# SelennLamson/AntsRL

Hardware: AMD Instinct MI355X
Metric: ant-steps/sec (ants x envs x steps/s), 256^2 grid (higher is better)
Workload: dtype f64 ant kinematics / f32 grids

## Files before the change

### antsrl_amd/_lib.py

```python
from __future__ import annotations

import ctypes as C
import os

from .config import AntsCfg, AntsGen, AntsInit

LIB_PATH = os.environ.get("ANTSRL_LIB") or os.path.join(os.path.dirname(os.path.abspath(__file__)), "lib",
                                                        "libantsrl_hip.so")

EXPORTS = ("antsrl_abi_version", "antsrl_cfg_size", "antsrl_last_error", "antsrl_workspace_bytes", "antsrl_create",
           "antsrl_destroy", "antsrl_reset", "antsrl_generate", "antsrl_step", "antsrl_observe", "antsrl_update", "antsrl_flush",
           "antsrl_step_update", "antsrl_set_timing_events", "antsrl_set_activation", "antsrl_policy_mlp", "antsrl_read_state", "antsrl_state_bytes",
           "antsrl_set_obs_format", "antsrl_query", "antsrl_bench_copy", "antsrl_set_inloop_policy", "antsrl_set_obs_row_stride", "antsrl_mem_alloc", "antsrl_mem_free",
           "antsrl_mem_trim", "antsrl_mem_stats", "antsrl_update_phase",
           "antsrl_perceptive_field", "antsrl_memnet_packed_bytes", "antsrl_memnet_pack", "antsrl_policy_memory",
           "antsrl_memtrain_sizes", "antsrl_memtrain_init", "antsrl_memtrain_unpack", "antsrl_memtrain_copy",
           "antsrl_memtrain_grad", "antsrl_memtrain_apply", "antsrl_memnet_packed_bytes_ex", "antsrl_memnet_pack_ex",
           "antsrl_policy_memory_ex", "antsrl_agent_select", "antsrl_replay_record_pre", "antsrl_replay_record_post",
           "antsrl_policy_memory_tiles", "antsrl_agent_plan", "antsrl_agent_select_actions",
           "antsrl_replay_record_pre_plain", "antsrl_replay_record_post_plain", "antsrl_lintrain_sizes",
           "antsrl_lintrain_grad", "antsrl_lintrain_apply", "antsrl_lintrain_step", "antsrl_exptrain_sizes",
           "antsrl_exptrain_grad", "antsrl_exptrain_apply", "antsrl_exptrain_step", "antsrl_rework_collapsed_bytes",
           "antsrl_rework_collapse", "antsrl_policy_rework", "antsrl_reworktrain_sizes", "antsrl_reworktrain_grad",
           "antsrl_reworktrain_apply", "antsrl_reworktrain_step", "antsrl_policy_rework_select", "antsrl_monitor_sizes",
           "antsrl_monitor_init", "antsrl_monitor_step", "antsrl_monitor_end_episode")

_lib = None


class AntsMemNetShape(C.Structure):
    _fields_ = [(n, C.c_int32) for n in ("n_features", "agent_dim", "mem_size", "h1", "h2", "h3", "n_rot", "n_ph")]


class AntsReworkShape(C.Structure):
    _fields_ = [(n, C.c_int32) for n in ("n_features", "agent_dim", "g1", "g2", "g3", "r1", "r2", "r3", "p1", "n_rot", "n_ph")]


class AntsRecordSpec(C.Structure):
    _fields_ = [(n, C.c_int32) for n in ("n_envs", "n_ants", "env_id_base", "n_features", "agent_dim", "mem_size", "n_rot",
                                         "obs_format", "obs_pitch", "reserved")] + [
        (n, C.c_int64) for n in ("K", "head", "max_len")] + [(n, C.c_uint64) for n in ("seed", "step")]


class AntsrlError(RuntimeError):
    pass


def load() -> C.CDLL:
    global _lib
    if _lib is not None:
        return _lib
    if not os.path.exists(LIB_PATH):
        raise AntsrlError(
            "libantsrl_hip.so is missing (%s): build it with `python -m antsrl_amd.build` "
            "(hipcc, gfx950).  There is no CPU fallback." % LIB_PATH)
    import torch
    lib = C.CDLL(LIB_PATH)
    vp, i32 = C.c_void_p, C.c_int
    lib.antsrl_abi_version.restype = i32
    lib.antsrl_last_error.restype = C.c_char_p
    lib.antsrl_workspace_bytes.argtypes = [C.POINTER(AntsCfg), C.POINTER(C.c_size_t)]
    lib.antsrl_create.argtypes = [C.POINTER(AntsCfg), vp, C.c_size_t, C.POINTER(vp)]
    lib.antsrl_destroy.argtypes = [vp]
    lib.antsrl_destroy.restype = None
    lib.antsrl_reset.argtypes = [vp, C.POINTER(AntsInit), vp]
    lib.antsrl_generate.argtypes = [vp, C.POINTER(AntsGen), C.c_uint64, vp]
    lib.antsrl_step.argtypes = [vp, vp, vp, vp, vp, vp, vp, vp]
    lib.antsrl_observe.argtypes = [vp, vp, vp, vp, vp]
    lib.antsrl_update.argtypes = [vp, vp, vp]
    lib.antsrl_flush.argtypes = [vp, vp]
    lib.antsrl_update_phase.argtypes = [vp, i32, vp, vp]
    lib.antsrl_perceptive_field.argtypes = [vp, vp, vp]
    lib.antsrl_step_update.argtypes = [vp, vp, vp, vp, vp, vp, vp, vp, vp]
    lib.antsrl_set_timing_events.argtypes = [vp, C.POINTER(vp)]
    lib.antsrl_set_activation.argtypes = [vp, vp, C.c_double, vp]
    lib.antsrl_policy_mlp.argtypes = [vp, vp, vp, C.c_int64, C.c_int32, vp, vp, vp, vp, vp, vp, vp, vp, vp, vp]
    lib.antsrl_read_state.argtypes = [vp, i32, vp, vp]
    lib.antsrl_state_bytes.argtypes = [vp, i32, C.POINTER(C.c_size_t)]
    lib.antsrl_query.argtypes = [vp, i32, C.POINTER(C.c_longlong)]
    lib.antsrl_set_inloop_policy.argtypes = [vp, i32] + [vp] * 9
    lib.antsrl_bench_copy.argtypes = [vp, vp, C.c_size_t, vp]
    lib.antsrl_set_obs_row_stride.argtypes = [vp, i32]
    lib.antsrl_mem_alloc.argtypes = [C.c_size_t, i32, C.POINTER(vp)]
    lib.antsrl_mem_free.argtypes = [vp]
    lib.antsrl_mem_trim.argtypes = []
    lib.antsrl_mem_stats.argtypes = [C.POINTER(C.c_size_t)] * 4
    lib.antsrl_memnet_packed_bytes.argtypes = [C.POINTER(AntsMemNetShape), C.POINTER(C.c_size_t)]
    lib.antsrl_memnet_pack.argtypes = [C.POINTER(AntsMemNetShape), C.POINTER(vp), vp, vp]
    lib.antsrl_policy_memory.argtypes = [C.POINTER(AntsMemNetShape), vp, vp, i32, vp, vp, C.c_int64, vp, vp, vp, vp, vp]
    lib.antsrl_memnet_packed_bytes_ex.argtypes = [C.POINTER(AntsMemNetShape), i32, C.POINTER(C.c_size_t)]
    lib.antsrl_memnet_pack_ex.argtypes = [C.POINTER(AntsMemNetShape), i32, C.POINTER(vp), vp, vp]
    lib.antsrl_policy_memory_ex.argtypes = [C.POINTER(AntsMemNetShape), i32, vp, vp, i32, vp, vp, C.c_int64, vp, vp, vp,
                                            vp, vp]
    lib.antsrl_policy_memory_tiles.argtypes = [C.POINTER(AntsMemNetShape), i32, vp, vp, i32, vp, vp, C.c_int64, vp, vp, vp,
                                               vp, vp, vp, vp]
# ... 100 lines not shown
```

### antsrl_amd/batched.py

```python
from __future__ import annotations

import ctypes as C
from typing import Dict, Optional

import numpy as np
import torch

from . import _lib
from . import config as cfgmod
from . import vmm
from .config import AntsCfg, AntsInit

_STATE_DTYPES = {
    cfgmod.S_ANTS_XYT: torch.float64, cfgmod.S_PREV_XY: torch.float64, cfgmod.S_HOLDING: torch.float32,
    cfgmod.S_MANDIBLES: torch.uint8, cfgmod.S_ACTIVATION: torch.float32, cfgmod.S_PHERO: torch.float32,
    cfgmod.S_FOOD: torch.float32, cfgmod.S_EXPLORED: torch.uint8, cfgmod.S_ANTHILL_FOOD: torch.float64,
    cfgmod.S_ROCK_CENTERS: torch.float64, cfgmod.S_TIMESTEP: torch.int32, cfgmod.S_REWARD_STATE: torch.uint8,
    cfgmod.S_WALLS: torch.uint8, cfgmod.S_ANTHILL_AREA: torch.uint8, cfgmod.S_SEED: torch.float32,
    cfgmod.S_ANTHILL_XYR: torch.int32, cfgmod.S_ROCK_RW: torch.float64,
    cfgmod.S_PHERO_C0: torch.float32, cfgmod.S_PHERO_C1: torch.float32, cfgmod.S_PHERO_C2: torch.float32,
    cfgmod.S_PHERO_C3: torch.float32,
}


import contextlib

_NULL_CTX = contextlib.nullcontext()
_RAW_STREAM = getattr(torch._C, "_cuda_getCurrentRawStream", None)


def _ptr(t: Optional[torch.Tensor]):
    return None if t is None else C.c_void_p(t.data_ptr())


def placement_levels_seen(times) -> bool:
    ok = [t for t in times if t < 1.25 * min(times)]
    return max(ok) >= 1.06 * min(ok)


class BatchedAntsEnv:
    def __init__(self, cfg: AntsCfg, device: Optional[torch.device] = None, obs_dtype: torch.dtype = torch.float32,
                 obs_row_stride=None, pieced_memory: bool = True):
        if obs_dtype not in (torch.float32, torch.bfloat16):
            raise ValueError("obs_dtype must be torch.float32 or torch.bfloat16")
        if not torch.cuda.is_available():
            raise _lib.AntsrlError("BatchedAntsEnv needs an MI355X (torch.cuda.is_available() is False); "
                                   "there is no CPU fallback")
        self.lib = _lib.load()
        self.cfg = cfg.copy()
        self.device = torch.device(device if device is not None else "cuda:%d" % torch.cuda.current_device())
        self._dev_index = self.device.index if self.device.index is not None else torch.cuda.current_device()
        need = C.c_size_t()
        _lib.check(self.lib.antsrl_workspace_bytes(C.byref(self.cfg), C.byref(need)), "workspace_bytes")
        self.workspace_bytes = need.value
        with torch.cuda.device(self.device):
            big = (lambda n: vmm.empty_u8(n, self.device)) if pieced_memory else (lambda n: torch.empty(n, dtype=torch.uint8, device=self.device))
            self._pieced = bool(pieced_memory)
            self._h = None
            self._make_handle(torch.empty(need.value + 256, dtype=torch.uint8, device=self.device))
            E, N, P, K = cfg.n_envs, cfg.n_ants, cfg.pside, cfg.n_channels
            esz = 4 if obs_dtype == torch.float32 else 2
            row = P * P * K
            if obs_row_stride not in (None, "line"):
                raise ValueError("obs_row_stride must be None or 'line'")
            pitch = row if obs_row_stride is None else (row * esz + 127) // 128 * 128 // esz
            sizes = [("agent_state", E * N * 2 * 4), ("reward", E * N * 4), ("done", E), ("obs", E * N * pitch * esz)]
            offs, total = {}, 0
            for name, nbytes in sizes:
                offs[name] = total
                total += (nbytes + 255) // 256 * 256
            self._out_sizes, self._out_offs, self._out_total, self._small_bytes = sizes, offs, total, offs["obs"]
            self._obs_dtype, self._obs_pitch_row = obs_dtype, (pitch, row)
            if obs_dtype == torch.bfloat16:
                _lib.check(self.lib.antsrl_set_obs_format(self._h, 1), "set_obs_format")
            if pitch != row:
                _lib.check(self.lib.antsrl_set_obs_row_stride(self._h, pitch), "set_obs_row_stride")
            self.obs_row_pitch = pitch
            self._bind_outputs(big(total + 256).zero_())
        self._keep = None
        self._loaded = None
        self._host_out = None
        self._host_act = None
        self._act_event = None

    def __del__(self):
        h = getattr(self, "_h", None)
        if h:
            self.lib.antsrl_destroy(h)
            self._h = None

    def _bind_outputs(self, flat: torch.Tensor) -> None:
        c = self.cfg
        E, N, P, K = c.n_envs, c.n_ants, c.pside, c.n_channels
        sizes, offs, total = self._out_sizes, self._out_offs, self._out_total
        pitch, row = self._obs_pitch_row
        base = (-flat.data_ptr()) % 256
        self._out_flat = flat[base:base + total]

        def piece(name, nbytes, dtype, shape):
            return self._out_flat[offs[name]:offs[name] + nbytes].view(dtype).view(shape)
        if pitch == row:
            self.obs = piece("obs", sizes[3][1], self._obs_dtype, (E, N, P, P, K))
            self.obs_padded = None
        else:
            self.obs_padded = piece("obs", sizes[3][1], self._obs_dtype, (E, N, pitch))
            self.obs = self.obs_padded[..., :row].unflatten(-1, (P, P, K))
        self.agent_state = piece("agent_state", sizes[0][1], torch.float32, (E, N, 2))
        self.reward = piece("reward", sizes[1][1], torch.float32, (E, N))
        self.done = piece("done", sizes[2][1], torch.uint8, (E,))
        self._host_out = None

    def _make_handle(self, ws: torch.Tensor) -> None:
        if getattr(self, "_h", None):
            self.lib.antsrl_destroy(self._h)
        self._ws = ws
        self._ws_ptr = ws.data_ptr() + (-ws.data_ptr()) % 256
        self._h = C.c_void_p()
        _lib.check(self.lib.antsrl_create(C.byref(self.cfg), C.c_void_p(self._ws_ptr), self.workspace_bytes, C.byref(self._h)), "create")
        if getattr(self, "_obs_dtype", torch.float32) == torch.bfloat16:
            _lib.check(self.lib.antsrl_set_obs_format(self._h, 1), "set_obs_format")
        pitch, row = getattr(self, "_obs_pitch_row", (0, 0))
        if pitch != row:
            _lib.check(self.lib.antsrl_set_obs_row_stride(self._h, pitch), "set_obs_row_stride")

    def tune_placement(self, age: int = 150, steps: int = 30, verbose: bool = False, extra_outputs: int = 4,
                       walk_spacers: int = 3, spacer_gib: float = 24.0, force_walk: bool = False):
        if self._out_total < vmm.SMALL_BYTES:
            return None
        if self._loaded:
            raise _lib.AntsrlError("tune_placement() must run right after construction: this handle has already been %s" % self._loaded)
        c = self.cfg
        E, N = c.n_envs, c.n_ants
        dev = self.device

        def torch_u8(n):
            return torch.empty(n, dtype=torch.uint8, device=dev)
        with torch.cuda.device(dev):
            g = torch.Generator(device=dev)
            g.manual_seed(7)
            rot = torch.randint(-1, 2, (4, E, N), generator=g, device=dev, dtype=torch.int8)
            ph = torch.randint(0, 3, (4, E, N), generator=g, device=dev, dtype=torch.int8) if c.n_phero == 2 else [None] * 4
            e0, e1 = torch.cuda.Event(enable_timing=True), torch.cuda.Event(enable_timing=True)

            def scratch_episode():
                self.generate(cfgmod.make_gen(), episode_seed=0x7A11)
                for t in range(age):
                    self.step_update(rot[t % 4], ph[t % 4], None)

            NEV, PSTEPS = cfgmod.TIMING_EVENTS, 8
            evs = _lib.HipEvents(NEV * PSTEPS)
            prc_times = []

            def measure():
                for t in range(4):
                    self.step_update(rot[t % 4], ph[t % 4], None)
                e0.record()
                for t in range(steps):
                    self.step_update(rot[t % 4], ph[t % 4], None)
                e1.record()
                for t in range(PSTEPS):
                    self.set_timing_events([evs.ev[NEV * t + i].value for i in range(NEV)])
                    self.step_update(rot[t % 4], ph[t % 4], None)
                torch.cuda.current_stream(dev).synchronize()
                prc_times.append(float(np.mean([evs.elapsed_ms(NEV * t + 2, NEV * t + 3) for t in range(PSTEPS)])))
                return e0.elapsed_time(e1) / steps
            own_ws, own_out = self._ws, self._out_flat
            n_ws, n_out = self.workspace_bytes + 256, self._out_total + 256
            pairs, times = [], []
            for ws_kind in ("own", "other"):
                if ws_kind == "other":
                    self._make_handle(vmm.empty_u8(n_ws, dev))
                scratch_episode()
                for out_kind in ("own", "other"):
                    if out_kind == "other":
                        self._bind_outputs((torch_u8(n_out) if self._pieced else vmm.empty_u8(n_out, dev)).zero_())
                    elif ws_kind == "other":
                        self._bind_outputs(own_out)
                    pairs.append((self._ws, self._out_flat))
                    times.append(measure())
            labels = ["ws torch / out %s" % ("pieced" if self._pieced else "torch"),
                      "ws torch / out %s" % ("torch" if self._pieced else "pieced"),
                      "ws pieced / out %s" % ("pieced" if self._pieced else "torch"),
                      "ws pieced / out %s" % ("torch" if self._pieced else "pieced")]
            if extra_outputs > 0 and self._pieced:
                self._make_handle(own_ws)
                scratch_episode()
                for k in range(int(extra_outputs)):
                    self._bind_outputs(vmm.empty_u8(n_out, dev).zero_())
                    pairs.append((self._ws, self._out_flat))
                    times.append(measure())
                    labels.append("ws torch / out pieced (draw %d)" % (k + 2))
            spacers = []
            walked = 0
            both_levels = placement_levels_seen
            while self._pieced and walked < int(walk_spacers) and (force_walk or not both_levels(prc_times)):
                free_b = torch.cuda.mem_get_info(dev)[0]
                want = int(min(spacer_gib * 2 ** 30, free_b / 5))
                if want < (4 << 30):
                    break
                try:
                    spacers.append(torch_u8(want))
                    spacers.append(vmm.empty_u8(want, dev))
                except (RuntimeError, _lib.AntsrlError):
                    break
                walked += 1
                depth = sum(x.numel() for x in spacers) / 2 ** 30
                if self._ws.data_ptr() != own_ws.data_ptr():
                    self._make_handle(own_ws)
                scratch_episode()
                for kind, mk in (("pieced", lambda: vmm.empty_u8(n_out, dev)), ("torch", lambda: torch_u8(n_out))):
                    self._bind_outputs(mk().zero_())
                    pairs.append((self._ws, self._out_flat))
                    times.append(measure())
                    labels.append("ws torch / out %s (walk %d: +%.0f GiB)" % (kind, walked, depth))
                self._make_handle(torch_u8(n_ws))
                scratch_episode()
                self._bind_outputs(own_out)
                pairs.append((self._ws, self._out_flat))
                times.append(measure())
                labels.append("ws torch (walk %d: +%.0f GiB) / out %s" % (walked, depth, "pieced" if self._pieced else "torch"))
            best = min(range(len(times)), key=prc_times.__getitem__)
            evs.destroy()
            if verbose:
                print("tune_placement: ms/step per (workspace, outputs) pair %s -> %d" % (["%.4f" % t for t in times], best))
            ws, out = pairs[best]
            del pairs, spacers
            if ws.data_ptr() != self._ws.data_ptr():
                self._make_handle(ws)
            self._bind_outputs(out)
            if walked:
                vmm.trim()
            torch.cuda.empty_cache()
            self._out_flat.zero_()
            del own_ws, own_out, ws, out
        self.placement_trials = dict(ms_per_step=[round(t, 5) for t in times], observation_kernel_ms=[round(t, 5) for t in prc_times],
                                     chosen=best, pairs=labels, both_levels_seen=bool(both_levels(prc_times)), walk_steps=walked)
        self._loaded = None
        return times

    @property
    def _obs_buf(self):
        return self.obs if self.obs_padded is None else self.obs_padded

    def _stream(self):
        if _RAW_STREAM is not None:
            return C.c_void_p(_RAW_STREAM(self._dev_index))
        return C.c_void_p(torch.cuda.current_stream(self.device).cuda_stream)

    def _on_device(self):
        return _NULL_CTX if torch.cuda.current_device() == self._dev_index else torch.cuda.device(self.device)

    def _dev(self, a, dtype, shape=None):
        if a is None:
            return None
        t = torch.as_tensor(np.ascontiguousarray(a) if isinstance(a, np.ndarray) else a)
        t = t.to(device=self.device, dtype=dtype).contiguous()
        if shape is not None:
            assert tuple(t.shape) == tuple(shape), "expected shape %s, got %s" % (shape, tuple(t.shape))
        return t

    def reset(self, init: Dict[str, object]) -> None:
        c = self.cfg
        E, N, W, H, Cn, R = c.n_envs, c.n_ants, c.w, c.h, c.n_phero, c.n_rocks
        t = dict(
            ants_xyt=self._dev(init["ants_xyt"], torch.float64, (E, N, 3)),
            seed=self._dev(init["seed"], torch.float64, (E, N)),
            walls=self._dev(init["walls"], torch.uint8, (E, W, H)),
            food=self._dev(init["food"], torch.float32, (E, W, H)),
            anthill_xyr=self._dev(init["anthill_xyr"], torch.int32, (E, 3)),
# ... 189 lines not shown
```

### antsrl_amd/csrc/antsrl_capi.hip

```cpp
#include <hip/hip_runtime.h>
#include <stdarg.h>
#include <stdio.h>
#include <math.h>
#include <stdlib.h>
#include <string.h>
#include <new>

#include "antsrl_device.h"
#include "antsrl_fail.h"

hipError_t antsrl_launch_act(const KP &p, const int8_t *rot, const int8_t *ph, int cur, float *obs,
                             float *agent_state, float *reward, uint8_t *done, int flags, hipStream_t st);
bool antsrl_act_fits(const KP &p);
bool antsrl_act_needs_hbm_maps(const KP &p);
hipError_t antsrl_launch_sweep(const KP &p, int cur, hipStream_t st);
hipError_t antsrl_launch_update(const KP &p, const double *jitter, int out_buf, hipStream_t st, int phases = 15);
hipError_t antsrl_launch_collect_full(const KP &p, hipStream_t st);
hipError_t antsrl_launch_reset(const KP &p, const AntsInit *in, hipStream_t st);
hipError_t antsrl_launch_set_activation(const KP &p, const float *act, hipStream_t st);
hipError_t antsrl_launch_read_state(const KP &p, int which, int cur, void *dst, hipStream_t st);
hipError_t antsrl_launch_perceptive_field(const KP &p, uint8_t *dst, hipStream_t st);
hipError_t antsrl_launch_generate(const KP &p, const AntsGen &g, uint64_t seed, hipStream_t st);
hipError_t antsrl_launch_phero_wall_clear(const KP &p, hipStream_t st, int buf = 0);
hipError_t antsrl_launch_phero_renorm(const KP &p, hipStream_t st);
bool antsrl_meta_supported(const KP &p);
hipError_t antsrl_launch_move(const KP &p, const int8_t *rot, const int8_t *ph, uint8_t *done, int do_step, uint32_t seq,
                              hipStream_t st);
hipError_t antsrl_launch_perceive(const KP &p, int cur, float *obs, float *agent_state, float *reward, int flags,
                                  uint32_t seq, hipStream_t st, const PolArgs *pol, uint32_t obs_pitch);
bool antsrl_inloop_policy_supported(const KP &p);
hipError_t antsrl_launch_policy_pack(unsigned char *pack, const float *w1, const float *b1, const float *w2, const float *b2,
                                     const float *w3, const float *b3, int F, hipStream_t st);
hipError_t antsrl_launch_meta_rebase(const KP &p, hipStream_t st);
bool antsrl_update_move_supported(const KP &p);
hipError_t antsrl_launch_update_move(const KP &p, int out_buf, double g_dep, double inv_g_dep, const int8_t *rot,
                                     const int8_t *ph, uint8_t *done, uint32_t seq, hipStream_t st, bool with_frames);
int antsrl_perceive_run(const KP &p);
hipError_t antsrl_launch_copy16(void *dst, const void *src, size_t bytes, hipStream_t st);

struct AntsHandle {
    AntsCfg cfg;
    KP p;
    int cur;
    int steps_since_update;
    bool need_full_collect;
    bool is_reset;
    bool episode_over;
    size_t ws_bytes;
    AntsGen gen;
    bool has_gen;
    uint64_t episode_seed;
    int host_timestep;
    long long sweeps;
    bool obs_bf16;
    uint32_t obs_pitch;
    bool need_wall_clear;
    hipEvent_t ev[ANTSRL_TIMING_EVENTS];
    bool ev_armed;
    uint32_t obs_seq;
    PolArgs pol;
    bool pend_update;
    KP pend_p;
    int pend_out_buf;
    int phase_next;
};

static thread_local char g_err[512] = "";

int fail(int code, const char *fmt, ...)
{
    va_list ap;
    va_start(ap, fmt);
    vsnprintf(g_err, sizeof(g_err), fmt, ap);
    va_end(ap);
    return code;
}

int hip_fail(hipError_t e, const char *what)
{
    return fail(ANTSRL_E_DEVICE, "%s: %s", what, hipGetErrorString(e));
}
// ... 34 lines not shown
    if (c->filter_radius < 0 || c->filter_radius > ANTSRL_MAX_FILTER_RADIUS)
        return fail(ANTSRL_E_INVALID, "filter_radius must be in 0..%d", ANTSRL_MAX_FILTER_RADIUS);
    if (c->reward_kind < ANTSRL_REWARD_NONE || c->reward_kind > ANTSRL_REWARD_ALL)
        return fail(ANTSRL_E_INVALID, "bad reward_kind");
    if (c->has_max_val && !(c->phero_max_val > 0)) return fail(ANTSRL_E_INVALID, "phero_max_val must be > 0");
    if (c->act_path < ANTSRL_ACT_AUTO || c->act_path > ANTSRL_ACT_SINGLE_KERNEL) return fail(ANTSRL_E_INVALID, "bad act_path");
    if (c->env_id_base < 0 || (long long)c->env_id_base + c->n_envs > 0x7fffffffll)
        return fail(ANTSRL_E_INVALID, "env_id_base must be >= 0 and env_id_base + n_envs must fit 31 bits");
    if (c->n_envs_total != 0 && (long long)c->n_envs_total < (long long)c->env_id_base + c->n_envs)
        return fail(ANTSRL_E_INVALID, "n_envs_total %d < env_id_base + n_envs = %lld (0 = that sum)", c->n_envs_total,
                    (long long)c->env_id_base + c->n_envs);
    if (c->act_path == ANTSRL_ACT_CELL_META) {
        KP kp;
        fill_kp(c, &kp);
        if (!kp.meta)
            return fail(ANTSRL_E_UNSUPPORTED, "ANTSRL_ACT_CELL_META needs 2 pheromone channels, the generator's channel order "
                                              "([Ants, Phero0, Phero1, Anthill, Walls, Food(, Rocks)]), a perception of 128..368 values "
                                              "per ant over at most 64 cells, and at most 4096 ants per env");
    }
    return ANTSRL_OK;
}

static bool use_scaled(const AntsCfg *c)
{
    return c->phero_mode == ANTSRL_PHERO_AUTO && c->filter_radius == 0 && c->filter[0] > 0.5 &&
           c->filter[0] <= 1.0 && c->phero_threshold >= 0.0;
}

static bool use_interleaved(const AntsCfg *c)
{
    return use_scaled(c) && c->n_phero == 2;
}

static size_t carve(const AntsCfg *c, DState *s, unsigned char *base)
{
    const size_t E = c->n_envs, N = c->n_ants, G = (size_t)c->w * c->h, Cn = c->n_phero, R = c->n_rocks;
    const size_t words = (G + 31) / 32;
    size_t off = 0;
    auto take = [&](size_t bytes) -> unsigned char * {
        unsigned char *ptr = base ? base + off : nullptr;
        off = (off + bytes + 255) / 256 * 256;
        return ptr;
    };
    KP kp;
    fill_kp(c, &kp);
    DState d;
    d.x = (double *)take(8 * E * N); d.y = (double *)take(8 * E * N); d.theta = (double *)take(8 * E * N);
    d.prev_x = (double *)take(8 * E * N); d.prev_y = (double *)take(8 * E * N);
    d.prev_dist = (double *)take(8 * E * N);
    d.holding = (float *)take(4 * E * N); d.seed = (float *)take(4 * E * N);
    d.prev_holding = (float *)take(4 * E * N);
    d.activation = (float *)take(4 * E * N * Cn);
    d.mandibles = (uint8_t *)take(E * N); d.reward_state = (uint8_t *)take(E * N);
    d.dirty_cell = (int32_t *)take(4 * E * N);
    d.walldep_cell = (int32_t *)take(4 * E * N);
    if (use_interleaved(c)) {
        d.phero[0] = d.phero[1] = (float *)take(16 * E * G);
        d.food = d.phero[0] ? d.phero[0] + 2 : nullptr;
    } else {
        d.phero[0] = (float *)take(4 * E * G * Cn);
        d.phero[1] = use_scaled(c) ? d.phero[0] : (float *)take(4 * E * G * Cn);
        d.food = (float *)take(4 * E * G * (size_t)kp.fs);
    }
    d.walls_bits = (uint32_t *)take(4 * E * words); d.area_bits = (uint32_t *)take(4 * E * words);
    d.explored_bits = (uint32_t *)take(4 * E * words);
    d.big_pres = d.big_old = nullptr;
    if (!kp.meta && antsrl_act_needs_hbm_maps(kp)) {
        d.big_pres = (uint32_t *)take(4 * E * words);
        d.big_old = (uint32_t *)take(4 * E * words);
    }
    d.primed_cur = kp.meta ? (uint8_t *)take(E) : nullptr;
    d.frames = kp.meta ? (AntFrame *)take(sizeof(AntFrame) * E * N) : nullptr;
    d.anthill_xyr = (int32_t *)take(4 * E * 3);
    d.anthill_food = (double *)take(8 * E);
    d.rock_cx = (double *)take(8 * E * (R ? R : 1)); d.rock_cy = (double *)take(8 * E * (R ? R : 1));
    d.rock_r = (double *)take(8 * E * (R ? R : 1)); d.rock_w = (double *)take(8 * E * (R ? R : 1));
    d.timestep = (int32_t *)take(4 * E);
    d.reward_primed = (uint8_t *)take(E);
    d.gen_discs = (int32_t *)take(4 * E * ANTSRL_MAX_FOOD_DISCS * 3);
    d.gen_perlin = (int32_t *)take(4 * E * 2);
    d.pol_pack = (unsigned char *)take(ANTSRL_POL_PACK_BYTES);
    if (s) *s = d;
    return off;
}

static void fill_kp(const AntsCfg *c, KP *p)
{
    memset(p, 0, sizeof(*p));
    p->E = c->n_envs; p->N = c->n_ants; p->W = c->w; p->H = c->h; p->C = c->n_phero; p->R = c->n_rocks;
    p->K = c->n_channels; p->r = c->perception_radius; p->P = 2 * p->r + 1; p->PP = p->P * p->P;
    p->words = (int)(((size_t)c->w * c->h + 31) / 32);
    int ht = 64;
    while (ht < 2 * c->n_ants) ht <<= 1;
    p->HT = ht;
    p->has_mask = c->has_mask; p->has_max_val = c->has_max_val; p->reward_kind = c->reward_kind;
    p->max_time = c->max_time; p->filter_radius = c->filter_radius;
    p->explore_on = c->reward_kind == ANTSRL_REWARD_EXPLORATION ||
                    (c->reward_kind == ANTSRL_REWARD_ALL &&
                     (c->fct_explore != 0.0 || c->fct_explore_holding != 0.0));
    for (int k = 0; k < ANTSRL_MAX_CHANNELS; ++k) {
        p->ch_kind[k] = c->channel_kind[k];
        p->ch_arg[k] = c->channel_arg[k];
    }
    p->mand_first = p->mand_last = 0;
    for (int k = 0; k < c->n_channels; ++k) {
        const int op = c->channel_kind[k] == ANTSRL_CH_FOOD ? 1 : c->channel_kind[k] == ANTSRL_CH_ANTHILL ? 2 : 0;
        if (op && op != p->mand_last) {
            p->mand_first = p->mand_last;
            p->mand_last = op;
        }
    }
    memcpy(p->mask, c->mask, ANTSRL_MAX_PCELLS);
    p->delta = c->delta; p->fwd_delta = c->fwd_delta; p->max_speed = c->max_speed;
    p->max_rot_speed = c->max_rot_speed; p->carry = c->carry_speed_reduction;
    p->backward = c->backward_speed_reduction; p->max_hold = c->max_hold;
    p->max_val = c->phero_max_val; p->deposit_strength = c->deposit_strength;
// ... 33 lines not shown
                    const float uh = (float)u[k], vh = (float)v[k];
                    p->fsep_u[2 * k] = uh; p->fsep_u[2 * k + 1] = (float)(u[k] - (double)uh);
                    p->fsep_v[2 * k] = vh; p->fsep_v[2 * k + 1] = (float)(v[k] - (double)vh);
                }
            }
        }
    }
    p->rng_seed = c->rng_seed;
    p->env_id_base = (uint32_t)c->env_id_base;
    p->scaled = use_scaled(c) ? 1 : 0;
    p->ps = use_interleaved(c) ? 4 : c->n_phero;
    p->fs = use_interleaved(c) ? 4 : 1;
    p->g_now = p->g_dep = p->inv_g_dep = 1.0;
    p->meta = antsrl_meta_supported(*p) && c->act_path != ANTSRL_ACT_SINGLE_KERNEL ? 1 : 0;
    if (p->meta && p->fs == 1) p->fs = 2;
    p->tiled = (p->meta && p->ps == 4 && p->fs == 4 && (c->w & 1) == 0 && (c->h & 3) == 0) ? 1 : 0;
    p->ftile = (p->meta && p->fs == 2 && (c->w & 3) == 0 && (c->h & 3) == 0) ? 1 : 0;
}

static void set_decay(AntsHandle *h)
{
    if (!h->p.scaled) return;
    const double f0 = h->cfg.filter[0];
    h->p.g_now = pow(f0, (double)h->sweeps);
    h->p.g_dep = pow(f0, (double)(h->sweeps + 1));
    h->p.inv_g_dep = 1.0 / h->p.g_dep;
}

extern "C" int antsrl_workspace_bytes(const AntsCfg *cfg, size_t *bytes)
{
    int rc = validate(cfg);
    if (rc) return rc;
    if (!bytes) return fail(ANTSRL_E_INVALID, "bytes is NULL");
    *bytes = carve(cfg, nullptr, nullptr);
    return ANTSRL_OK;
}

extern "C" int antsrl_create(const AntsCfg *cfg, void *workspace, size_t workspace_bytes, AntsHandle **out)
{
    int rc = validate(cfg);
    if (rc) return rc;
    if (!out) return fail(ANTSRL_E_INVALID, "out is NULL");
    if (!workspace) return fail(ANTSRL_E_INVALID, "workspace is NULL");
    if (((uintptr_t)workspace & 255) != 0) return fail(ANTSRL_E_INVALID, "workspace must be 256-byte aligned");
    const size_t need = carve(cfg, nullptr, nullptr);
    if (workspace_bytes < need)
        return fail(ANTSRL_E_NOMEM, "workspace too small: %zu < %zu bytes", workspace_bytes, need);
    AntsHandle *h = new (std::nothrow) AntsHandle();
    if (!h) return fail(ANTSRL_E_NOMEM, "out of host memory");
    h->cfg = *cfg;
    fill_kp(cfg, &h->p);
    carve(cfg, &h->p.s, (unsigned char *)workspace);
    h->cur = 0; h->steps_since_update = 0; h->need_full_collect = true; h->is_reset = false; h->episode_over = false; h->pend_update = false;
    h->phase_next = 0;
    h->pol = PolArgs{};
    h->sweeps = 0; h->need_wall_clear = false;
    h->has_gen = false; h->episode_seed = 0; h->host_timestep = 1; h->obs_bf16 = false; h->obs_pitch = 0;
    h->ws_bytes = need;
    h->ev_armed = false;
    h->obs_seq = 0;
    if (!h->p.meta && !antsrl_act_fits(h->p)) {
        delete h;
        return fail(ANTSRL_E_UNSUPPORTED,
                    "%d ants with a %dx%d perception need more than 160 KiB of LDS per workgroup "
                    "(per-ant frames, the collision hash and the row staging are kept in LDS)", cfg->n_ants,
                    2 * cfg->perception_radius + 1, 2 * cfg->perception_radius + 1);
    }
    *out = h;
    return ANTSRL_OK;
}

extern "C" void antsrl_destroy(AntsHandle *h) { delete h; }

extern "C" int antsrl_reset(AntsHandle *h, const AntsInit *init, void *stream)
{
    if (!h || !init) return fail(ANTSRL_E_INVALID, "NULL handle or init");
    if (!init->ants_xyt || !init->seed || !init->walls || !init->food || !init->anthill_xyr)
        return fail(ANTSRL_E_INVALID, "AntsInit: ants_xyt, seed, walls, food, anthill_xyr are required");
    if (h->p.R > 0 && !init->rocks) return fail(ANTSRL_E_INVALID, "AntsInit.rocks is NULL but n_rocks > 0");
    h->pend_update = false;
    h->phase_next = 0;
    hipError_t e = antsrl_launch_reset(h->p, init, (hipStream_t)stream);
    if (e != hipSuccess) return hip_fail(e, "reset");
    h->p.deposit_strength = h->cfg.deposit_strength;
    h->cur = 0; h->steps_since_update = 0; h->need_full_collect = true; h->is_reset = true; h->episode_over = false;
    h->sweeps = 0; h->need_wall_clear = h->p.scaled && init->phero != nullptr;
    h->host_timestep = 1; h->obs_seq = 0;
    set_decay(h);
    return ANTSRL_OK;
}

static int check_gen_seed(const AntsHandle *h, const AntsGen &g, uint64_t seed)
{
    const uint64_t top = (uint64_t)h->p.env_id_base + (uint64_t)h->p.E;
    const uint64_t lim = 0xFFFFFFFFull / 5u;
    if (g.rng_kind == ANTSRL_RNG_REFERENCE && (top > lim || seed > lim - top))
        return fail(ANTSRL_E_INVALID, "ANTSRL_RNG_REFERENCE: (episode_seed + env_id_base + n_envs) * 5 must stay below 2^32 (np.random.seed)");
    return ANTSRL_OK;
}

static int do_generate(AntsHandle *h, uint64_t seed, hipStream_t st)
{
// ... 500 lines not shown
```

### include/antsrl.h

```cpp
#ifndef ANTSRL_H
#define ANTSRL_H

#include <stddef.h>
#include <stdint.h>

#ifdef __cplusplus
extern "C" {
#endif

#define ANTSRL_ABI_VERSION 5

#define ANTSRL_MAX_CHANNELS 16
#define ANTSRL_MAX_PSIDE 15
#define ANTSRL_MAX_PCELLS (ANTSRL_MAX_PSIDE * ANTSRL_MAX_PSIDE)
#define ANTSRL_MAX_FILTER_RADIUS 3
#define ANTSRL_MAX_FILTER_TAPS 49
#define ANTSRL_MAX_PHERO 4

#define ANTSRL_OK 0
#define ANTSRL_E_INVALID (-1)
#define ANTSRL_E_NOMEM (-2)
#define ANTSRL_E_DEVICE (-3)
#define ANTSRL_E_UNSUPPORTED (-4)

// ... 98 lines not shown
    ANTSRL_S_PREV_XY = 1,
    ANTSRL_S_HOLDING = 2,
    ANTSRL_S_MANDIBLES = 3,
    ANTSRL_S_ACTIVATION = 4,
    ANTSRL_S_PHERO = 5,
    ANTSRL_S_FOOD = 6,
    ANTSRL_S_EXPLORED = 7,
    ANTSRL_S_ANTHILL_FOOD = 8,
    ANTSRL_S_ROCK_CENTERS = 9,
    ANTSRL_S_TIMESTEP = 10,
    ANTSRL_S_REWARD_STATE = 11,
    ANTSRL_S_WALLS = 12,
    ANTSRL_S_ANTHILL_AREA = 13,
    ANTSRL_S_SEED = 14,
    ANTSRL_S_ANTHILL_XYR = 15,
    ANTSRL_S_ROCK_RW = 16,
    ANTSRL_S_PHERO_C0 = 17,
    ANTSRL_S_PHERO_C1 = 18,
    ANTSRL_S_PHERO_C2 = 19,
    ANTSRL_S_PHERO_C3 = 20,
    ANTSRL_S_COUNT_
};

int antsrl_abi_version(void);

size_t antsrl_cfg_size(void);

const char *antsrl_last_error(void);

int antsrl_workspace_bytes(const AntsCfg *cfg, size_t *bytes);

int antsrl_create(const AntsCfg *cfg, void *workspace, size_t workspace_bytes, AntsHandle **out);

void antsrl_destroy(AntsHandle *h);

int antsrl_reset(AntsHandle *h, const AntsInit *init, void *stream);

int antsrl_generate(AntsHandle *h, const AntsGen *gen, uint64_t episode_seed, void *stream);

int antsrl_step(AntsHandle *h, const int8_t *rotation, const int8_t *phero, float *obs,
                float *agent_state, float *reward, uint8_t *done, void *stream);

int antsrl_observe(AntsHandle *h, float *obs, float *agent_state, float *reward, void *stream);

int antsrl_update(AntsHandle *h, const double *wall_jitter, void *stream);

enum { ANTSRL_PHASE_WALLS = 0, ANTSRL_PHASE_ROCKS_PHEROMONE = 1, ANTSRL_PHASE_ANTS = 2, ANTSRL_PHASE_ANTHILL = 3 };
int antsrl_update_phase(AntsHandle *h, int phase, const double *wall_jitter, void *stream);

int antsrl_flush(AntsHandle *h, void *stream);

int antsrl_step_update(AntsHandle *h, const int8_t *rotation, const int8_t *phero,
                       const double *wall_jitter, float *obs, float *agent_state, float *reward,
                       uint8_t *done, void *stream);

#define ANTSRL_TIMING_EVENTS 5
int antsrl_set_timing_events(AntsHandle *h, void *const *events);

enum {
    ANTSRL_Q_CELL_META = 0,
    ANTSRL_Q_SCALED_UNITS = 1,
    ANTSRL_Q_INTERLEAVED = 2,
    ANTSRL_Q_FILTER_SEPARABLE = 3,
    ANTSRL_Q_PERCEIVE_RUN = 4,
    ANTSRL_Q_TIMESTEP = 5,
    ANTSRL_Q_DEFERRED_UPDATE = 6,
// ... 197 lines not shown
```

Baseline: 2.678 billion.

## Split workspace into separate state and record blocks with tuned placement

Splits the device workspace into two allocations: a small per-ant and per-env state block, and a large record block holding the pheromone and food grids. tune_placement gains a second stage that times alternative placements of the state block (default torch, pieced VMM, or spare record-block candidates). It keeps one only if the update kernel gets faster by a margin. The aim is to cut memory-placement interference between small state arrays and the large grid arrays. It adds API surface and tuning time, and the choice rests on noisy measurements.

```diff
diff --git a/antsrl_amd/_lib.py b/antsrl_amd/_lib.py
--- a/antsrl_amd/_lib.py
+++ b/antsrl_amd/_lib.py
@@ -9,6 +9,7 @@
                                                         "libantsrl_hip.so")
 
 EXPORTS = ("antsrl_abi_version", "antsrl_cfg_size", "antsrl_last_error", "antsrl_workspace_bytes", "antsrl_create",
+           "antsrl_workspace_map",
            "antsrl_destroy", "antsrl_reset", "antsrl_generate", "antsrl_step", "antsrl_observe", "antsrl_update", "antsrl_flush",
            "antsrl_step_update", "antsrl_set_timing_events", "antsrl_set_activation", "antsrl_policy_mlp", "antsrl_read_state", "antsrl_state_bytes",
            "antsrl_set_obs_format", "antsrl_query", "antsrl_bench_copy", "antsrl_set_inloop_policy", "antsrl_set_obs_row_stride", "antsrl_mem_alloc", "antsrl_mem_free",
@@ -42,6 +43,10 @@
         (n, C.c_int64) for n in ("K", "head", "max_len")] + [(n, C.c_uint64) for n in ("seed", "step")]
 
 
+class AntsWsArray(C.Structure):
+    _fields_ = [("name", C.c_char * 24), ("block", C.c_int32), ("_pad", C.c_int32), ("offset", C.c_uint64), ("bytes", C.c_uint64)]
+
+
 class AntsrlError(RuntimeError):
     pass
 
@@ -61,6 +66,9 @@
     lib.antsrl_last_error.restype = C.c_char_p
     lib.antsrl_workspace_bytes.argtypes = [C.POINTER(AntsCfg), C.POINTER(C.c_size_t)]
     lib.antsrl_create.argtypes = [C.POINTER(AntsCfg), vp, C.c_size_t, C.POINTER(vp)]
+    lib.antsrl_workspace_bytes2.argtypes = [C.POINTER(AntsCfg), C.POINTER(C.c_size_t), C.POINTER(C.c_size_t)]
+    lib.antsrl_create2.argtypes = [C.POINTER(AntsCfg), vp, C.c_size_t, vp, C.c_size_t, C.POINTER(vp)]
+    lib.antsrl_workspace_map.argtypes = [C.POINTER(AntsCfg), i32, C.POINTER(AntsWsArray), C.c_int32, C.POINTER(C.c_int32)]
     lib.antsrl_destroy.argtypes = [vp]
     lib.antsrl_destroy.restype = None
     lib.antsrl_reset.argtypes = [vp, C.POINTER(AntsInit), vp]
diff --git a/antsrl_amd/batched.py b/antsrl_amd/batched.py
--- a/antsrl_amd/batched.py
+++ b/antsrl_amd/batched.py
@@ -40,7 +40,7 @@
 
 class BatchedAntsEnv:
     def __init__(self, cfg: AntsCfg, device: Optional[torch.device] = None, obs_dtype: torch.dtype = torch.float32,
-                 obs_row_stride=None, pieced_memory: bool = True):
+                 obs_row_stride=None, pieced_memory: bool = True, split_workspace: bool = True):
         if obs_dtype not in (torch.float32, torch.bfloat16):
             raise ValueError("obs_dtype must be torch.float32 or torch.bfloat16")
         if not torch.cuda.is_available():
@@ -53,11 +53,18 @@
         need = C.c_size_t()
         _lib.check(self.lib.antsrl_workspace_bytes(C.byref(self.cfg), C.byref(need)), "workspace_bytes")
         self.workspace_bytes = need.value
+        nst, nrec = C.c_size_t(), C.c_size_t()
+        _lib.check(self.lib.antsrl_workspace_bytes2(C.byref(self.cfg), C.byref(nst), C.byref(nrec)), "workspace_bytes2")
+        self.state_bytes, self.record_bytes = nst.value, nrec.value
+        self._split = bool(split_workspace)
+        if not self._split:
+            self.state_bytes, self.record_bytes = 0, self.workspace_bytes
         with torch.cuda.device(self.device):
             big = (lambda n: vmm.empty_u8(n, self.device)) if pieced_memory else (lambda n: torch.empty(n, dtype=torch.uint8, device=self.device))
             self._pieced = bool(pieced_memory)
             self._h = None
-            self._make_handle(torch.empty(need.value + 256, dtype=torch.uint8, device=self.device))
+            self._state = None
+            self._make_handle(torch.empty(self.record_bytes + 256, dtype=torch.uint8, device=self.device))
             E, N, P, K = cfg.n_envs, cfg.n_ants, cfg.pside, cfg.n_channels
             esz = 4 if obs_dtype == torch.float32 else 2
             row = P * P * K
@@ -110,13 +117,26 @@
         self.done = piece("done", sizes[2][1], torch.uint8, (E,))
         self._host_out = None
 
-    def _make_handle(self, ws: torch.Tensor) -> None:
+    def _make_handle(self, ws: torch.Tensor, state: Optional[torch.Tensor] = None) -> None:
         if getattr(self, "_h", None):
             self.lib.antsrl_destroy(self._h)
-        self._ws = ws
+            self._h = None
+        if ws.numel() < self.record_bytes + (-ws.data_ptr()) % 256:
+            raise _lib.AntsrlError("record block too small: %d bytes for %d" % (ws.numel(), self.record_bytes))
         self._ws_ptr = ws.data_ptr() + (-ws.data_ptr()) % 256
         self._h = C.c_void_p()
-        _lib.check(self.lib.antsrl_create(C.byref(self.cfg), C.c_void_p(self._ws_ptr), self.workspace_bytes, C.byref(self._h)), "create")
+        if not self._split:
+            self._ws, self._state = ws, None
+            _lib.check(self.lib.antsrl_create(C.byref(self.cfg), C.c_void_p(self._ws_ptr), self.workspace_bytes, C.byref(self._h)), "create")
+        else:
+            if state is None:
+                state = self._state if self._state is not None else torch.empty(self.state_bytes + 256, dtype=torch.uint8, device=self.device)
+            if state.numel() < self.state_bytes + (-state.data_ptr()) % 256:
+                raise _lib.AntsrlError("state block too small: %d bytes for %d" % (state.numel(), self.state_bytes))
+            self._ws, self._state = ws, state
+            self._state_ptr = state.data_ptr() + (-state.data_ptr()) % 256
+            _lib.check(self.lib.antsrl_create2(C.byref(self.cfg), C.c_void_p(self._state_ptr), self.state_bytes,
+                                               C.c_void_p(self._ws_ptr), self.record_bytes, C.byref(self._h)), "create2")
         if getattr(self, "_obs_dtype", torch.float32) == torch.bfloat16:
             _lib.check(self.lib.antsrl_set_obs_format(self._h, 1), "set_obs_format")
         pitch, row = getattr(self, "_obs_pitch_row", (0, 0))
@@ -124,7 +144,7 @@
             _lib.check(self.lib.antsrl_set_obs_row_stride(self._h, pitch), "set_obs_row_stride")
 
     def tune_placement(self, age: int = 150, steps: int = 30, verbose: bool = False, extra_outputs: int = 4,
-                       walk_spacers: int = 3, spacer_gib: float = 24.0, force_walk: bool = False):
+                       walk_spacers: int = 3, spacer_gib: float = 24.0, force_walk: bool = False, state_stage: bool = True):
         if self._out_total < vmm.SMALL_BYTES:
             return None
         if self._loaded:
@@ -147,25 +167,27 @@
                 for t in range(age):
                     self.step_update(rot[t % 4], ph[t % 4], None)
 
-            NEV, PSTEPS = cfgmod.TIMING_EVENTS, 8
-            evs = _lib.HipEvents(NEV * PSTEPS)
+            NEV, PSTEPS, PSTEPS_STATE = cfgmod.TIMING_EVENTS, 8, 24
+            evs = _lib.HipEvents(NEV * PSTEPS_STATE)
             prc_times = []
-
-            def measure():
+            upd_times = []
+
+            def measure(psteps=PSTEPS):
                 for t in range(4):
                     self.step_update(rot[t % 4], ph[t % 4], None)
                 e0.record()
                 for t in range(steps):
                     self.step_update(rot[t % 4], ph[t % 4], None)
                 e1.record()
-                for t in range(PSTEPS):
+                for t in range(psteps):
                     self.set_timing_events([evs.ev[NEV * t + i].value for i in range(NEV)])
                     self.step_update(rot[t % 4], ph[t % 4], None)
                 torch.cuda.current_stream(dev).synchronize()
-                prc_times.append(float(np.mean([evs.elapsed_ms(NEV * t + 2, NEV * t + 3) for t in range(PSTEPS)])))
+                prc_times.append(float(np.mean([evs.elapsed_ms(NEV * t + 2, NEV * t + 3) for t in range(psteps)])))
+                upd_times.append(float(np.mean([evs.elapsed_ms(NEV * t + 1, NEV * t + 2) for t in range(psteps)])))
                 return e0.elapsed_time(e1) / steps
-            own_ws, own_out = self._ws, self._out_flat
-            n_ws, n_out = self.workspace_bytes + 256, self._out_total + 256
+            own_ws, own_out, own_state = self._ws, self._out_flat, self._state
+            n_ws, n_out, n_state = self.record_bytes + 256, self._out_total + 256, self.state_bytes + 256
             pairs, times = [], []
             for ws_kind in ("own", "other"):
                 if ws_kind == "other":
@@ -220,21 +242,52 @@
                 times.append(measure())
                 labels.append("ws torch (walk %d: +%.0f GiB) / out %s" % (walked, depth, "pieced" if self._pieced else "torch"))
             best = min(range(len(times)), key=prc_times.__getitem__)
-            evs.destroy()
             if verbose:
                 print("tune_placement: ms/step per (workspace, outputs) pair %s -> %d" % (["%.4f" % t for t in times], best))
             ws, out = pairs[best]
-            del pairs, spacers
-            if ws.data_ptr() != self._ws.data_ptr():
-                self._make_handle(ws)
+            n_stage1 = len(times)
+            state_cands = [("state torch (default)", own_state)]
+            if state_stage and self._split:
+                try:
+                    state_cands.append(("state pieced", vmm.pieced_u8(n_state, dev)))
+                except _lib.AntsrlError:
+                    pass
+                seen = {ws.data_ptr()}
+                for (w2, _o), lab in zip(pairs, labels):
+                    if w2.data_ptr() not in seen and w2.numel() >= n_state and len(state_cands) < 4:
+                        seen.add(w2.data_ptr())
+                        state_cands.append(("state in spare record block (%s)" % lab.split(" / ")[0], w2[:n_state]))
+            for lab, st in state_cands if len(state_cands) > 1 else []:
+                self._make_handle(ws, st)
+                self._bind_outputs(out)
+                scratch_episode()
+                times.append(measure(PSTEPS_STATE))
+            evs.destroy()
+            s_upd, s_prc = upd_times[n_stage1:], prc_times[n_stage1:]
+            times, prc_times, upd_times = times[:n_stage1], prc_times[:n_stage1], upd_times[:n_stage1]
+            s_best = 0
+            if s_upd:
+                def fast(k, by):
+                    return s_upd[k] <= (1.0 - by) * s_upd[0] and s_upd[k] + s_prc[k] < s_upd[0] + s_prc[0]
+                own = [k for k in range(1, len(s_upd)) if state_cands[k][0] == "state pieced" and fast(k, 0.03)]
+                corners = [k for k in range(1, len(s_upd)) if state_cands[k][0] != "state pieced" and fast(k, 0.05)]
+                if own or corners:
+                    s_best = min(own or corners, key=s_upd.__getitem__)
+            state = state_cands[s_best][1]
+            state_labels = [lab for lab, _ in state_cands]
+            del pairs, spacers, state_cands
+            if ws.data_ptr() != self._ws.data_ptr() or (state is not None and state.data_ptr() != self._state.data_ptr()):
+                self._make_handle(ws, state)
             self._bind_outputs(out)
             if walked:
                 vmm.trim()
             torch.cuda.empty_cache()
             self._out_flat.zero_()
-            del own_ws, own_out, ws, out
+            del own_ws, own_out, own_state, ws, out, state
         self.placement_trials = dict(ms_per_step=[round(t, 5) for t in times], observation_kernel_ms=[round(t, 5) for t in prc_times],
-                                     chosen=best, pairs=labels, both_levels_seen=bool(both_levels(prc_times)), walk_steps=walked)
+                                     chosen=best, pairs=labels, both_levels_seen=bool(both_levels(prc_times)), walk_steps=walked,
+                                     state_stage=dict(candidates=state_labels, update_move_kernel_ms=[round(t, 5) for t in s_upd],
+                                                      observation_kernel_ms=[round(t, 5) for t in s_prc], chosen=s_best))
         self._loaded = None
         return times
 
diff --git a/antsrl_amd/csrc/antsrl_capi.hip b/antsrl_amd/csrc/antsrl_capi.hip
--- a/antsrl_amd/csrc/antsrl_capi.hip
+++ b/antsrl_amd/csrc/antsrl_capi.hip
@@ -46,7 +46,7 @@
     bool need_full_collect;
     bool is_reset;
     bool episode_over;
-    size_t ws_bytes;
+    size_t ws_bytes[2];
     AntsGen gen;
     bool has_gen;
     uint64_t episode_seed;
@@ -147,56 +147,70 @@
     return use_scaled(c) && c->n_phero == 2;
 }
 
-static size_t carve(const AntsCfg *c, DState *s, unsigned char *base)
+static void carve(const AntsCfg *c, DState *s, unsigned char *base, unsigned char *rec_base, bool split, size_t bytes[2],
+                  AntsWsArray *map = nullptr, int32_t cap = 0, int32_t *count = nullptr)
 {
     const size_t E = c->n_envs, N = c->n_ants, G = (size_t)c->w * c->h, Cn = c->n_phero, R = c->n_rocks;
     const size_t words = (G + 31) / 32;
-    size_t off = 0;
-    auto take = [&](size_t bytes) -> unsigned char * {
-        unsigned char *ptr = base ? base + off : nullptr;
-        off = (off + bytes + 255) / 256 * 256;
+    size_t off[2] = {0, 0};
+    int32_t n_arrays = 0;
+    auto take_from = [&](int block, const char *name, size_t nbytes) -> unsigned char * {
+        unsigned char *b = block ? rec_base : base;
+        size_t &o = off[split ? block : 0];
+        unsigned char *ptr = b ? b + o : nullptr;
+        if (map && n_arrays < cap) {
+            AntsWsArray &a = map[n_arrays];
+            memset(&a, 0, sizeof(a));
+            strncpy(a.name, name, sizeof(a.name) - 1);
+            a.block = split ? block : 0; a.offset = o; a.bytes = nbytes;
+        }
+        ++n_arrays;
+        o = (o + nbytes + 255) / 256 * 256;
         return ptr;
     };
+    auto take = [&](const char *name, size_t nbytes) { return take_from(0, name, nbytes); };
+    auto take_rec = [&](const char *name, size_t nbytes) { return take_from(1, name, nbytes); };
     KP kp;
     fill_kp(c, &kp);
     DState d;
-    d.x = (double *)take(8 * E * N); d.y = (double *)take(8 * E * N); d.theta = (double *)take(8 * E * N);
-    d.prev_x = (double *)take(8 * E * N); d.prev_y = (double *)take(8 * E * N);
-    d.prev_dist = (double *)take(8 * E * N);
-    d.holding = (float *)take(4 * E * N); d.seed = (float *)take(4 * E * N);
-    d.prev_holding = (float *)take(4 * E * N);
-    d.activation = (float *)take(4 * E * N * Cn);
-    d.mandibles = (uint8_t *)take(E * N); d.reward_state = (uint8_t *)take(E * N);
-    d.dirty_cell = (int32_t *)take(4 * E * N);
-    d.walldep_cell = (int32_t *)take(4 * E * N);
+    d.x = (double *)take("x", 8 * E * N); d.y = (double *)take("y", 8 * E * N); d.theta = (double *)take("theta", 8 * E * N);
+    d.prev_x = (double *)take("prev_x", 8 * E * N); d.prev_y = (double *)take("prev_y", 8 * E * N);
+    d.prev_dist = (double *)take("prev_dist", 8 * E * N);
+    d.holding = (float *)take("holding", 4 * E * N); d.seed = (float *)take("seed", 4 * E * N);
+    d.prev_holding = (float *)take("prev_holding", 4 * E * N);
+    d.activation = (float *)take("activation", 4 * E * N * Cn);
+    d.mandibles = (uint8_t *)take("mandibles", E * N); d.reward_state = (uint8_t *)take("reward_state", E * N);
+    d.dirty_cell = (int32_t *)take("dirty_cell", 4 * E * N);
+    d.walldep_cell = (int32_t *)take("walldep_cell", 4 * E * N);
     if (use_interleaved(c)) {
-        d.phero[0] = d.phero[1] = (float *)take(16 * E * G);
+        d.phero[0] = d.phero[1] = (float *)take_rec("records", 16 * E * G);
         d.food = d.phero[0] ? d.phero[0] + 2 : nullptr;
     } else {
-        d.phero[0] = (float *)take(4 * E * G * Cn);
-        d.phero[1] = use_scaled(c) ? d.phero[0] : (float *)take(4 * E * G * Cn);
-        d.food = (float *)take(4 * E * G * (size_t)kp.fs);
-    }
-    d.walls_bits = (uint32_t *)take(4 * E * words); d.area_bits = (uint32_t *)take(4 * E * words);
-    d.explored_bits = (uint32_t *)take(4 * E * words);
+        d.phero[0] = (float *)take_rec("phero0", 4 * E * G * Cn);
+        d.phero[1] = use_scaled(c) ? d.phero[0] : (float *)take_rec("phero1", 4 * E * G * Cn);
+        d.food = (float *)take_rec("food", 4 * E * G * (size_t)kp.fs);
+    }
+    d.walls_bits = (uint32_t *)take("walls_bits", 4 * E * words); d.area_bits = (uint32_t *)take("area_bits", 4 * E * words);
+    d.explored_bits = (uint32_t *)take("explored_bits", 4 * E * words);
     d.big_pres = d.big_old = nullptr;
     if (!kp.meta && antsrl_act_needs_hbm_maps(kp)) {
-        d.big_pres = (uint32_t *)take(4 * E * words);
-        d.big_old = (uint32_t *)take(4 * E * words);
-    }
-    d.primed_cur = kp.meta ? (uint8_t *)take(E) : nullptr;
-    d.frames = kp.meta ? (AntFrame *)take(sizeof(AntFrame) * E * N) : nullptr;
-    d.anthill_xyr = (int32_t *)take(4 * E * 3);
-    d.anthill_food = (double *)take(8 * E);
-    d.rock_cx = (double *)take(8 * E * (R ? R : 1)); d.rock_cy = (double *)take(8 * E * (R ? R : 1));
-    d.rock_r = (double *)take(8 * E * (R ? R : 1)); d.rock_w = (double *)take(8 * E * (R ? R : 1));
-    d.timestep = (int32_t *)take(4 * E);
-    d.reward_primed = (uint8_t *)take(E);
-    d.gen_discs = (int32_t *)take(4 * E * ANTSRL_MAX_FOOD_DISCS * 3);
-    d.gen_perlin = (int32_t *)take(4 * E * 2);
-    d.pol_pack = (unsigned char *)take(ANTSRL_POL_PACK_BYTES);
+        d.big_pres = (uint32_t *)take("big_pres", 4 * E * words);
+        d.big_old = (uint32_t *)take("big_old", 4 * E * words);
+    }
+    d.primed_cur = kp.meta ? (uint8_t *)take("primed_cur", E) : nullptr;
+    d.frames = kp.meta ? (AntFrame *)take("frames", sizeof(AntFrame) * E * N) : nullptr;
+    d.anthill_xyr = (int32_t *)take("anthill_xyr", 4 * E * 3);
+    d.anthill_food = (double *)take("anthill_food", 8 * E);
+    d.rock_cx = (double *)take("rock_cx", 8 * E * (R ? R : 1)); d.rock_cy = (double *)take("rock_cy", 8 * E * (R ? R : 1));
+    d.rock_r = (double *)take("rock_r", 8 * E * (R ? R : 1)); d.rock_w = (double *)take("rock_w", 8 * E * (R ? R : 1));
+    d.timestep = (int32_t *)take("timestep", 4 * E);
+    d.reward_primed = (uint8_t *)take("reward_primed", E);
+    d.gen_discs = (int32_t *)take("gen_discs", 4 * E * ANTSRL_MAX_FOOD_DISCS * 3);
+    d.gen_perlin = (int32_t *)take("gen_perlin", 4 * E * 2);
+    d.pol_pack = (unsigned char *)take("pol_pack", ANTSRL_POL_PACK_BYTES);
     if (s) *s = d;
-    return off;
+    if (count) *count = n_arrays;
+    bytes[0] = off[0]; bytes[1] = off[1];
 }
 
 static void fill_kp(const AntsCfg *c, KP *p)
@@ -296,31 +310,48 @@
     int rc = validate(cfg);
     if (rc) return rc;
     if (!bytes) return fail(ANTSRL_E_INVALID, "bytes is NULL");
-    *bytes = carve(cfg, nullptr, nullptr);
-    return ANTSRL_OK;
-}
-
-extern "C" int antsrl_create(const AntsCfg *cfg, void *workspace, size_t workspace_bytes, AntsHandle **out)
+    size_t b[2];
+    carve(cfg, nullptr, nullptr, nullptr, false, b);
+    *bytes = b[0];
+    return ANTSRL_OK;
+}
+
+extern "C" int antsrl_workspace_bytes2(const AntsCfg *cfg, size_t *state_bytes, size_t *record_bytes)
 {
     int rc = validate(cfg);
     if (rc) return rc;
-    if (!out) return fail(ANTSRL_E_INVALID, "out is NULL");
-    if (!workspace) return fail(ANTSRL_E_INVALID, "workspace is NULL");
-    if (((uintptr_t)workspace & 255) != 0) return fail(ANTSRL_E_INVALID, "workspace must be 256-byte aligned");
-    const size_t need = carve(cfg, nullptr, nullptr);
-    if (workspace_bytes < need)
-        return fail(ANTSRL_E_NOMEM, "workspace too small: %zu < %zu bytes", workspace_bytes, need);
+    size_t b[2];
+    carve(cfg, nullptr, nullptr, nullptr, true, b);
+    if (state_bytes) *state_bytes = b[0];
+    if (record_bytes) *record_bytes = b[1];
+    return ANTSRL_OK;
+}
+
+extern "C" int antsrl_workspace_map(const AntsCfg *cfg, int split, AntsWsArray *entries, int32_t cap, int32_t *count)
+{
+    int rc = validate(cfg);
+    if (rc) return rc;
+    if (!count) return fail(ANTSRL_E_INVALID, "count is NULL");
+    if (cap < 0 || (cap > 0 && !entries)) return fail(ANTSRL_E_INVALID, "entries is NULL or cap < 0");
+    size_t b[2];
+    carve(cfg, nullptr, nullptr, nullptr, split != 0, b, entries, cap, count);
+    return ANTSRL_OK;
+}
+
+static int create_handle(const AntsCfg *cfg, void *state_ws, void *record_ws, bool split, const size_t need[2], AntsHandle **out)
+{
     AntsHandle *h = new (std::nothrow) AntsHandle();
     if (!h) return fail(ANTSRL_E_NOMEM, "out of host memory");
     h->cfg = *cfg;
     fill_kp(cfg, &h->p);
-    carve(cfg, &h->p.s, (unsigned char *)workspace);
+    size_t b[2];
+    carve(cfg, &h->p.s, (unsigned char *)state_ws, (unsigned char *)record_ws, split, b);
     h->cur = 0; h->steps_since_update = 0; h->need_full_collect = true; h->is_reset = false; h->episode_over = false; h->pend_update = false;
     h->phase_next = 0;
     h->pol = PolArgs{};
     h->sweeps = 0; h->need_wall_clear = false;
     h->has_gen = false; h->episode_seed = 0; h->host_timestep = 1; h->obs_bf16 = false; h->obs_pitch = 0;
-    h->ws_bytes = need;
+    h->ws_bytes[0] = need[0]; h->ws_bytes[1] = need[1];
     h->ev_armed = false;
     h->obs_seq = 0;
     if (!h->p.meta && !antsrl_act_fits(h->p)) {
@@ -332,6 +363,41 @@
     }
     *out = h;
     return ANTSRL_OK;
+}
+
+extern "C" int antsrl_create(const AntsCfg *cfg, void *workspace, size_t workspace_bytes, AntsHandle **out)
+{
+    int rc = validate(cfg);
+    if (rc) return rc;
+    if (!out) return fail(ANTSRL_E_INVALID, "out is NULL");
+    if (!workspace) return fail(ANTSRL_E_INVALID, "workspace is NULL");
+    if (((uintptr_t)workspace & 255) != 0) return fail(ANTSRL_E_INVALID, "workspace must be 256-byte aligned");
+    size_t need[2];
+    carve(cfg, nullptr, nullptr, nullptr, false, need);
+    if (workspace_bytes < need[0])
+        return fail(ANTSRL_E_NOMEM, "workspace too small: %zu < %zu bytes", workspace_bytes, need[0]);
+    return create_handle(cfg, workspace, workspace, false, need, out);
+}
+
+extern "C" int antsrl_create2(const AntsCfg *cfg, void *state_ws, size_t state_bytes, void *record_ws, size_t record_bytes,
+                              AntsHandle **out)
+{
+    int rc = validate(cfg);
+    if (rc) return rc;
+    if (!out) return fail(ANTSRL_E_INVALID, "out is NULL");
+    if (!state_ws || !record_ws) return fail(ANTSRL_E_INVALID, "state_ws or record_ws is NULL");
+    if ((((uintptr_t)state_ws | (uintptr_t)record_ws) & 255) != 0)
+        return fail(ANTSRL_E_INVALID, "state_ws and record_ws must be 256-byte aligned");
+    size_t need[2];
+    carve(cfg, nullptr, nullptr, nullptr, true, need);
+    if (state_bytes < need[0])
+        return fail(ANTSRL_E_NOMEM, "state block too small: %zu < %zu bytes", state_bytes, need[0]);
+    if (record_bytes < need[1])
+        return fail(ANTSRL_E_NOMEM, "record block too small: %zu < %zu bytes", record_bytes, need[1]);
+    const uintptr_t s0 = (uintptr_t)state_ws, r0 = (uintptr_t)record_ws;
+    if (s0 < r0 + need[1] && r0 < s0 + need[0])
+        return fail(ANTSRL_E_INVALID, "the state block and the record block overlap");
+    return create_handle(cfg, state_ws, record_ws, true, need, out);
 }
 
 extern "C" void antsrl_destroy(AntsHandle *h) { delete h; }
diff --git a/include/antsrl.h b/include/antsrl.h
--- a/include/antsrl.h
+++ b/include/antsrl.h
@@ -154,6 +154,17 @@
 
 int antsrl_create(const AntsCfg *cfg, void *workspace, size_t workspace_bytes, AntsHandle **out);
 
+int antsrl_workspace_bytes2(const AntsCfg *cfg, size_t *state_bytes, size_t *record_bytes);
+int antsrl_create2(const AntsCfg *cfg, void *state_ws, size_t state_bytes, void *record_ws, size_t record_bytes,
+                   AntsHandle **out);
+
+typedef struct AntsWsArray {
+    char name[24];
+    int32_t block, _pad;
+    uint64_t offset, bytes;
+} AntsWsArray;
+int antsrl_workspace_map(const AntsCfg *cfg, int split, AntsWsArray *entries, int32_t cap, int32_t *count);
+
 void antsrl_destroy(AntsHandle *h);
 
 int antsrl_reset(AntsHandle *h, const AntsInit *init, void *stream);
```

New measurement: 2.708 billion (median of 6 runs). 1.01x the previous value.
